# jytime/Deep-SfM-Revisited

Measured on AMD Instinct MI355X. Metric: image-pairs/sec (5-pt RANSAC + nlabel=128 plane-sweep), KITTI 376×1242, higher is better.
Workload: dtype f64+f32; 1 GPU; KITTI 376x1242 dense flow (N=435032, read by the RANSAC kernels), H=4096 hypotheses (ransac_iter=8), nlabel=128, C=32 at 94x311, fp32 cost volume; pairs_per_gpu=8, global_batch=8, parallelism=dp1, streams=one stream

## Files before the change

### deep-sfm-revisited_amd/csrc/ransac5.hip

```cpp
#include <string>
#include <vector>
#include "ransac_common.h"

namespace sfm {

template <class Src>
static int run_chunk(const Src& src, const int64_t* n, int bc, int num_test,
                     int num_ransac_test, int iters, double thr, uint64_t seed, int cheir,
                     const Workspace& w, int ws_batch, double* E_out, double* P_out, int32_t* inliers_out,
                     int32_t* winner_out, int32_t* score_out, hipStream_t s, bool first_chunk,
                     const RefJob* ref_job = nullptr, bool* rode = nullptr) {
  const int H = kChains * iters;
  const int cmax = H * kMaxSlots;
  PairParams pp{};
  for (int b = 0; b < bc; ++b) {
    pp.n[b] = n[b];
    pp.test[b] = (int32_t)(num_test > 0 ? num_test : n[b]);
    pp.rtest[b] = (int32_t)(num_ransac_test > 0 ? num_ransac_test : n[b]);
    const int M = std::max(pp.test[b], pp.rtest[b]);
    pp.splits[b] = (M + kPtsPerItem - 1) / kPtsPerItem;
  }
  const ScorePlan plan = make_score_plan(thr, pp, bc, cmax, ws_batch, score_out != nullptr, true);
  launch_solve(src, pp, bc, H, seed, cheir, w, s);
  SFM_LAUNCHED();
// ... 158 lines not shown
    set_error("workspace too small: need " + std::to_string(need) + " bytes");
    return SFM_ERR_WORKSPACE;
  }
  hipStream_t s = (hipStream_t)stream;
  char* p = (char*)workspace;
  const size_t c = (size_t)batch * ncand;
  ScoreBufs w;
  w.cand_total = (int32_t*)p;
  p += align_up(SFM_MAX_BATCH * 4);
  w.candE = (double*)p;
  p += align_up(c * kCandStride * 8);
  w.candF = (_Float16*)p;
  p += align_up(c * kMfRec * 2);
  w.cntR = (int32_t*)p;
  p += align_up(c * 4);
  w.claim = (unsigned long long*)p;
  w.cntT = counts;
  PairParams pp{};
  for (int b = 0; b < batch; ++b) {
    pp.n[b] = n[b];
    pp.test[b] = pp.rtest[b] = (int32_t)n[b];
    pp.splits[b] = (int32_t)((n[b] + kPtsPerItem - 1) / kPtsPerItem);
  }
  const ScorePlan plan = make_score_plan(thr, pp, batch, ncand, batch, false, false);
  SFM_HIP(hipMemsetAsync(w.cntT, 0, c * 4, s));
  SFM_HIP(hipMemsetAsync(w.cntR, 0, c * 4, s));
  launch_fill_cands(E, batch, ncand, thr, plan, w, s);
  ProfScope ps("score_essentials", s);
  launch_score(PackedSrc{pts, n_stride}, pp, w, plan, s);
  SFM_LAUNCHED();
  return SFM_OK;
}

int sfm_ransac5_candidate_counts(const void* workspace, size_t workspace_bytes, int batch, int iters,
                                 int32_t* counts_host) {
  SFM_REQUIRE(workspace && counts_host && batch >= 1 && batch <= SFM_MAX_BATCH && iters >= 1, "invalid arguments");
  const int bc = batch;
  SFM_REQUIRE(workspace_bytes >= layout(nullptr, bc, 0, iters, nullptr), "workspace too small");
  Workspace w;
  layout((char*)workspace, bc, 0, iters, &w);
  SFM_HIP(hipMemcpy(counts_host, w.cand_total, sizeof(int32_t) * batch, hipMemcpyDeviceToHost));
  return SFM_OK;
}

int sfm_ransac5_hypothesis_counts(const void* workspace, size_t workspace_bytes, int batch, int iters,
                                  int32_t* nroots_host, int32_t* ncand_host) {
  SFM_REQUIRE(workspace && nroots_host && ncand_host && batch >= 1 && batch <= SFM_MAX_BATCH && iters >= 1,
              "invalid arguments");
  const int bc = batch;
  SFM_REQUIRE(workspace_bytes >= layout(nullptr, bc, 0, iters, nullptr), "workspace too small");
  Workspace w;
  layout((char*)workspace, bc, 0, iters, &w);
  const size_t bytes = sizeof(int32_t) * (size_t)batch * kChains * iters;
  SFM_HIP(hipMemcpy(nroots_host, w.nroots, bytes, hipMemcpyDeviceToHost));
  SFM_HIP(hipMemcpy(ncand_host, w.ncand, bytes, hipMemcpyDeviceToHost));
  return SFM_OK;
}

int sfm_ransac5_skipped_evaluations(const void* workspace, size_t workspace_bytes, int batch, int iters,
                                    unsigned long long* skipped_host) {
  SFM_REQUIRE(workspace && skipped_host && batch >= 1 && iters >= 1, "invalid arguments");
  const int bc = std::min(batch, SFM_MAX_BATCH);
  SFM_REQUIRE(workspace_bytes >= layout(nullptr, bc, 0, iters, nullptr), "workspace too small");
  Workspace w;
  layout((char*)workspace, bc, 0, iters, &w);
  SFM_HIP(hipMemcpy(skipped_host, w.skipped, sizeof(unsigned long long), hipMemcpyDeviceToHost));
// ... 19 lines not shown
```

### deep-sfm-revisited_amd/csrc/ransac_common.h

```cpp
#pragma once
#include <algorithm>
#include "common.h"

namespace sfm {

constexpr int kChains = SFM_RANSAC_CHAINS;
constexpr int kMaxSlots = 10;
constexpr size_t kMf2ClaimBytes = 9 * sizeof(unsigned long long);
constexpr int kCandStride = 18;
constexpr int kStEb = 0, kStA = 36, kStQ = 75, kStPoly = 95, kStRoots = 106, kStateFields = 116;
constexpr int kKC = 32;
constexpr int kPPL = 8;
constexpr int kScoreThreads = 256;
constexpr int kChunk = kScoreThreads * kPPL;
constexpr int kPPL32 = 8;
constexpr int kPtsPerItem = 8192;
static_assert(kPtsPerItem % kChunk == 0, "item = whole chunks");
constexpr int kMfRec = 64;
constexpr int kMf2Span = 1024;
constexpr int kBestStride = 64;

struct PairParams {
  int64_t n[SFM_MAX_BATCH];
  int32_t test[SFM_MAX_BATCH];
// ... 153 lines not shown
  int32_t* cmap = nullptr;
  int32_t* lead = nullptr;
  unsigned long long* skipped = nullptr;
  int32_t* bnd = nullptr;
};

struct MfParams {
  int k;
  double t_lo, t_hi;
};

enum class Scorer {
  kMf2Prune,
  kMf2,
  kMf,
  kLowp,
  kScore32,
  kFma,
  kRef
};
struct ScorePlan {
  Scorer scorer;
  int bc, cmax;
  bool same;
  int prec;
  ScoreConsts kc;
  MfParams mp;
  double guard_g;
  bool fast32;
  int cus;
  int grid;
  int mf2_pm;
  bool one_cnt;
};
#pragma GCC visibility push(hidden)
ScorePlan make_score_plan(double thr, const PairParams& pp, int bc, int cmax, int ws_batch, bool want_scores,
                          bool allow_prune);
template <class Src>
void launch_score(const Src& src, const PairParams& pp, const ScoreBufs& w, const ScorePlan& plan, hipStream_t s,
                  const RefJob* ref_job = nullptr, bool* rode = nullptr);

template <class Src>
void launch_solve(const Src& src, const PairParams& pp, int bc, int H, uint64_t seed, int cheir, const Workspace& w,
                  hipStream_t s);
void launch_chain(int bc, int H, int iters, int cheir, double thr, const ScorePlan& plan, const Workspace& w,
                  bool first_chunk, hipStream_t s);
void launch_select(int bc, int H, int cheir, const ScorePlan& plan, const Workspace& w, int32_t* score_out,
                   double* E_out, double* P_out, int32_t* inliers_out, int32_t* winner_out, hipStream_t s);
void launch_fill_cands(const double* E, int batch, int ncand, double thr, const ScorePlan& plan, const ScoreBufs& w,
                       hipStream_t s);
#pragma GCC visibility pop

}
```

### deep-sfm-revisited_amd/csrc/ransac_score.hip

```cpp
#include "score_mf2.h"

namespace sfm {

template <int kFmt>
static bool make_rider(const RefJob& j, long long max_runs, RefRider<kFmt>* r) {
  const long long hw = (long long)j.h * j.w, L = j.nlabel;
  const long long esz = kFmt == 1 ? 4 : 2;
  if (hw < 4 || hw % 2 != 0 || (hw % 4 != 0 && L % 2 != 0)) return false;
  const long long P = hw % 4 == 0 ? hw : 2 * hw, np = L * hw / P;
  const long long slab_bytes = L * hw * esz;
  if (slab_bytes >= (1ll << 32) || (uintptr_t)j.ref % 8 != 0 || (uintptr_t)j.cost % 16 != 0) return false;
  const long long rows = (long long)j.batch * j.channels;
  const long long cpp = (P + 255) / 256, gpp = (np + kRiderStores - 1) / kRiderStores;
  const long long T = rows * cpp * gpp;
  if (T >= (1ll << 31) || max_runs >= (1ll << 31)) return false;
  r->ref = j.ref;
  r->cost = j.cost;
  r->T = (unsigned)T;
  r->C = (unsigned)j.channels;
  r->hw = (unsigned)hw;
  r->P = (unsigned)P;
  r->cpp = (unsigned)cpp;
  r->np = (unsigned)np;
  r->gpp = (unsigned)gpp;
// ... 2 lines not shown
  r->mgpp = make_magic((unsigned)gpp);
  r->mC = make_magic((unsigned)j.channels);
  return true;
}

static int lowp_prec() {
  const int p = tuning().score_precision;
  return (p != 64 && tuning().score_lowp_template) ? p + 1 : p;
}

ScorePlan make_score_plan(double thr, const PairParams& pp, int bc, int cmax, int ws_batch, bool want_scores,
                          bool allow_prune) {
  ScorePlan p{};
  p.bc = bc;
  p.cmax = cmax;
  p.prec = lowp_prec();
  const bool fast = p.prec == 64 && thr >= 0x1p-40 && thr < 1.0;
  p.guard_g = fast ? 0x1p24 * (11.0 + 11.0 / thr) : 0.0;
  p.fast32 = fast && thr >= 0x1p-20 && tuning().score_fp32;
  ScoreConsts& kc = p.kc;
  kc.thr = thr;
  kc.t2lo = (thr * thr) * (1.0 - 0x1p-22);
  kc.t2hi = (thr * thr) * (1.0 + 0x1p-22);
  kc.t2lo32 = (float)((thr * thr) * (1.0 - 0x1p-6 - 0x1p-19));
  kc.t2hi32 = (float)((thr * thr) * (1.0 + 0x1p-7) / (1.0 - 0x1p-7) * (1.0 + 0x1p-19));
  kc.fast32 = p.fast32 ? 1 : 0;
  kc.ws_batch = ws_batch;
  kc.interleave = tuning().score_interleave;
  int dev = 0, cus = 256;
  if (hipGetDevice(&dev) == hipSuccess) (void)hipDeviceGetAttribute(&cus, hipDeviceAttributeMultiprocessorCount, dev);
  p.cus = std::max(1, cus);
  p.grid = p.cus * tuning().score_blocks_per_cu;
  p.same = true;
  int min_spans = INT32_MAX;
  for (int b = 0; b < bc; ++b) {
    p.same = p.same && pp.test[b] == pp.rtest[b];
    min_spans = std::min(min_spans, mf2_spans(std::max(pp.test[b], pp.rtest[b])));
  }
  const bool use_mf = p.fast32 && tuning().score_mf && mf_params(thr, &p.mp);
  const bool mf2 = use_mf && p.same && tuning().score_mf == 2;
  const bool may_prune = allow_prune && p.same && !want_scores;
  kc.prune = (p.fast32 && !use_mf && may_prune && tuning().score_prune) ? 1 : 0;
  p.mf2_pm = (mf2 && may_prune && min_spans >= kMf2PruneMinSpans) ? tuning().score_mf_prune : 0;
  p.one_cnt = mf2;
  const bool lowp = p.prec == 32 || p.prec == 16 || p.prec == 33 || p.prec == 17;
  p.scorer = mf2 ? (p.mf2_pm > 0 ? Scorer::kMf2Prune : Scorer::kMf2)
             : use_mf ? Scorer::kMf
             : lowp ? Scorer::kLowp
             : p.fast32 ? Scorer::kScore32
             : fast ? Scorer::kFma
                    : Scorer::kRef;
  return p;
}

struct Mf2Launch {
  const int32_t* cand_total;
  const int32_t* cmap;
  int sp_lo, sp_hi;
  const int32_t* bnd;
  int phase;
  int chunk;
};
static Mf2Launch spans_pm(const int32_t* cand_total, int lo, int hi, int chunk, const int32_t* cmap = nullptr) {
  return Mf2Launch{cand_total, cmap, lo, hi, nullptr, 0, chunk};
}
static Mf2Launch spans_bnd(const int32_t* cand_total, const int32_t* bnd, int phase, int chunk,
                           const int32_t* cmap = nullptr) {
  return Mf2Launch{cand_total, cmap, 0, 0, bnd, phase, chunk};
}

template <class Src, bool kMapped, bool kUpper, class... Rider>
// ... 4 lines not shown
                     a.sp_lo, a.sp_hi, a.bnd, a.phase, a.chunk, rider...);
}

template <int kFmt, class Src>
static bool try_ride(const Src& src, const PairParams& pp, const ScoreBufs& w, const ScorePlan& plan, hipStream_t s,
                     const Mf2Launch& a, const RefJob* job, long long max_runs) {
  RefRider<kFmt> r;
  if (!job || !tuning().score_ref_rider || job->dtype != kFmt - 1 || !make_rider(*job, max_runs, &r)) return false;
  launch_mf2<Src, false, true>(src, pp, w, plan, s, a, r);
  return true;
}

template <class Src, bool kUpper>
static void launch_mf2_pruned(const Src& src, const PairParams& pp, const ScoreBufs& w, const ScorePlan& plan,
                              hipStream_t s, const RefJob* ref_job, bool* rode) {
  const int bc = plan.bc, cmax = plan.cmax;
  const int ch = tuning().score_mf_chunk;
  const int ch2 = tuning().score_mf_chunk2 ? tuning().score_mf_chunk2 : ch;
  const int32_t* kept = w.lead + 3 * SFM_MAX_BATCH;
  const Mf2Launch A = spans_pm(w.cand_total, 0, plan.mf2_pm, ch);
  bool ride = false;
  if constexpr (kUpper) {
    long long max_runs = 0;
    for (int b = 0; b < bc; ++b)
      max_runs += (long long)mf2_spans(std::max(pp.test[b], pp.rtest[b])) * ((cmax + kKC - 1) / kKC);
    ride = try_ride<1>(src, pp, w, plan, s, A, ref_job, max_runs) ||
           try_ride<2>(src, pp, w, plan, s, A, ref_job, max_runs);
    if (ride) *rode = true;
  }
  if (!ride) launch_mf2<Src, false, kUpper>(src, pp, w, plan, s, A);
  hipLaunchKernelGGL(k_mf2_split, dim3(bc), dim3(1024), 0, s, pp, cmax, plan.mf2_pm, tuning().score_mf_prune_margin,
                     w.cand_total, w.cntT, w.bnd, kUpper ? w.lead : nullptr);
  launch_mf2<Src, false, kUpper>(src, pp, w, plan, s, spans_bnd(w.cand_total, w.bnd, 1, ch));
  hipLaunchKernelGGL(k_mf2_lead<Src>, dim3(kUpper ? 4 * kLeadBlocks : kLeadBlocks, bc), dim3(1024), 0, s, src, pp,
                     cmax, w.bnd, w.cand_total, w.candE, w.cntT, plan.kc, w.lead, kUpper ? 2 : 0);
  hipLaunchKernelGGL(k_mf2_keep, dim3((cmax + 1023) / 1024, bc), dim3(1024), 0, s, pp, cmax, w.bnd, w.cand_total,
                     w.cntT, w.lead, w.cmap, w.skipped, 0);
  launch_mf2<Src, true, kUpper>(src, pp, w, plan, s, spans_bnd(kept, w.bnd, 2, ch2, w.cmap));
  if constexpr (kUpper) {
    const int exact_max = tuning().score_mf_exact_max;
    hipLaunchKernelGGL(k_mf2_keep_map, dim3(bc), dim3(1024), 0, s, cmax, w.cntT, w.lead, w.cmap, w.cmap2, exact_max);
    hipLaunchKernelGGL(k_mf2_zero_kept, dim3((cmax + 255) / 256, bc), dim3(256), 0, s, cmax, w.lead, w.cmap2, w.cntT);
    hipLaunchKernelGGL(k_mf2_exact<Src>, dim3(kExactBlocks, bc), dim3(kExactThreads), 0, s, src, pp, cmax, w.lead,
                       w.cmap2, w.candE, plan.kc, w.cntT, exact_max);
    launch_mf2<Src, true, false>(src, pp, w, plan, s, spans_pm(w.lead + 4 * SFM_MAX_BATCH, 0, 1000, ch2, w.cmap2));
  }
}

template <bool FAST, int PREC, class Src>
static void launch_valu(const Src& src, const PairParams& pp, const ScoreBufs& w, const ScorePlan& plan,
                        hipStream_t s, const char* name) {
  hipLaunchKernelGGL((k_score<FAST, Src, PREC>), dim3(plan.grid), dim3(kScoreThreads), 0, s, src, pp, plan.bc,
                     plan.cmax, w.cand_total, w.candE, w.cntT, w.cntR, plan.kc);
  set_last_scorer(name);
}

template <class Src>
void launch_score(const Src& src, const PairParams& pp, const ScoreBufs& w, const ScorePlan& plan, hipStream_t s,
                  const RefJob* ref_job, bool* rode) {
  const int bc = plan.bc, cmax = plan.cmax;
  if (plan.scorer <= Scorer::kMf)
    hipLaunchKernelGGL(k_mf_cands, dim3((cmax + 255) / 256, bc), dim3(256), 0, s, cmax, w.cand_total, w.candE, w.candF,
                       plan.mp, w.claim, plan.mf2_pm > 0 ? w.lead : nullptr);
  const dim3 gmf(plan.cus * tuning().score_mf_blocks_per_cu);
  switch (plan.scorer) {
    case Scorer::kMf2Prune:
      if (tuning().score_mf_prune_upper) launch_mf2_pruned<Src, true>(src, pp, w, plan, s, ref_job, rode);
      else launch_mf2_pruned<Src, false>(src, pp, w, plan, s, ref_job, rode);
      set_last_scorer("k_score_mf2+prune");
      break;
    case Scorer::kMf2:
      launch_mf2<Src, false, false>(src, pp, w, plan, s, spans_pm(w.cand_total, 0, 1000, tuning().score_mf_chunk));
      set_last_scorer("k_score_mf2");
      break;
    case Scorer::kMf:
      if (plan.same)
        hipLaunchKernelGGL((k_score_mf<Src, true>), gmf, dim3(kMfWaves * 64), 0, s, src, pp, bc, cmax, w.cand_total,
                           w.candE, w.candF, w.cntT, w.cntR, plan.kc);
      else
// ... 31 lines not shown
```

### deep-sfm-revisited_amd/csrc/score_mf2.h

```cpp
#pragma once
#include <hip/hip_bf16.h>
#include "score_mf.h"

namespace sfm {

constexpr int kMf2Waves = 12;
constexpr int kMf2Wpe = kMf2Waves / 4;
#ifndef SFM_MF2_UP_WAVES
#define SFM_MF2_UP_WAVES 16
#endif
template <bool kUpper> constexpr int mf2_waves() { return kUpper ? SFM_MF2_UP_WAVES : kMf2Waves; }
constexpr int kMf2Tiles = kMf2Span / 32;
constexpr int kMf2Guide = 2;
constexpr int kMf2Queue = 128;
#ifndef SFM_MF2_WQ
#define SFM_MF2_WQ 1
#endif
constexpr int kMf2WordSlots = kMf2Queue / 2;
constexpr int kMf2TblTiles = 352;
constexpr int kMf2TblWords = kMf2TblTiles * kKC / 2;
constexpr int kMf2TblSpans = 63;
constexpr int kMf2PruneMinSpans = 32;
static_assert(kMf2Span <= 1024, "16-bit table counts");
static_assert(kMf2Tiles <= 32 && kMf2Tiles % 2 == 0, "32-bit decision strings, tiles in pairs");
// ... 485 lines not shown
        if constexpr (kRide) {
          __builtin_amdgcn_s_waitcnt(0x0F70);
          if (rp < rp_end) {
            const auto& rj = rider_of(rider...);
            rider_store(rj, rp, lane, rd);
            for (unsigned p = rp + 1u; p < rp_end; ++p) rider_store(rj, p, lane, rider_load(rj, p, lane));
          }
        }
        k = kn;
      }
      u += k1 - k0;
      lds_barrier();
    }
  }
  if (tb >= 0) flush(tb);
  __syncthreads();
  if (tid == 0) {
    __threadfence();
    if (atomicAdd(claim + 8, 1ull) == (unsigned long long)G - 1ull) {
#pragma unroll
      for (int i = 0; i < 9; ++i) claim[i] = 0ull;
    }
  }
}

constexpr int kLeadBlocks = 32;
constexpr int kExactMaxKept = 256;

__device__ __forceinline__ int mf2_n1(const PairParams& pp, int b, const int32_t* bnd) {
  const int M = max(pp.test[b], pp.rtest[b]);
  return min(bnd[2 * SFM_MAX_BATCH + b] * kMf2Span, M);
}

__global__ __launch_bounds__(1024) void k_mf2_split(PairParams pp, int cmax, int pm, int margin,
                                                   const int32_t* __restrict__ cand_total,
                                                   const int32_t* __restrict__ cntT, int32_t* __restrict__ bnd,
                                                   int32_t* __restrict__ leader) {
  __shared__ unsigned long long s_key[16];
  const int b = blockIdx.x, tid = threadIdx.x, lane = tid & 63, wv = tid >> 6;
  const int M = max(pp.test[b], pp.rtest[b]);
  const int all = mf2_spans(M);
  const int sA = mf2_span_at(all, pm);
  const int nA = min(sA * kMf2Span, M);
  const int ctot = cand_total[b];
  const int32_t* cnt = cntT + (size_t)b * cmax;
  unsigned long long key = 0ull;
  for (int c = tid; c < ctot; c += 1024) {
    const unsigned long long k = ((unsigned long long)(uint32_t)cnt[c] << 32) | (uint32_t)(0xFFFFFFFFu - (uint32_t)c);
    key = k > key ? k : key;
  }
#pragma unroll
  for (int d = 32; d >= 1; d >>= 1) {
    const unsigned long long o = __shfl_xor(key, d, 64);
    key = o > key ? o : key;
  }
  if (lane == 0) s_key[wv] = key;
  __syncthreads();
  if (tid != 0) return;
  for (int w = 0; w < 16; ++w) key = s_key[w] > key ? s_key[w] : key;
  int mx = (int)(key >> 32);
  if (leader && ctot > 0) {
    leader[0 * SFM_MAX_BATCH + b] = 0;
    leader[1 * SFM_MAX_BATCH + b] = (int)(0xFFFFFFFFu - (uint32_t)(key & 0xFFFFFFFFull));
  }
  const long long rho_pm = nA > 0 ? ((long long)mx * 1000) / nA : 0;
  long long f = 1000 - rho_pm + margin;
  f = max(f, (long long)pm);
  const int sB = f > 990 ? all : max(sA, mf2_span_at(all, (int)f));
  bnd[0 * SFM_MAX_BATCH + b] = 0;
  bnd[1 * SFM_MAX_BATCH + b] = sA;
  bnd[2 * SFM_MAX_BATCH + b] = sB;
  bnd[3 * SFM_MAX_BATCH + b] = all;
}

template <class Src>
__global__ __launch_bounds__(1024) void k_mf2_lead(const Src src, PairParams pp, int cmax, const int32_t* __restrict__ bnd,
                                                  const int32_t* __restrict__ cand_total,
                                                  const double* __restrict__ candE, const int32_t* __restrict__ cntT,
                                                  ScoreConsts kc, int32_t* __restrict__ lead, int full) {
  __shared__ unsigned long long s_key[16];
  __shared__ int s_part[16];
  const int b = blockIdx.y, tid = threadIdx.x, lane = tid & 63, wv = tid >> 6;
  const int M = max(pp.test[b], pp.rtest[b]);
  const int n1 = full ? 0 : mf2_n1(pp, b, bnd);
  const int ctot = cand_total[b];
  if (ctot <= 0) return;
  const int32_t* cnt = cntT + (size_t)b * cmax;
  if (full == 2) {
    const int ldr = lead[1 * SFM_MAX_BATCH + b];
    const int k0 = (int)((long long)M * blockIdx.x / gridDim.x);
    const int k1 = (int)((long long)M * (blockIdx.x + 1) / gridDim.x);
    const double* El = candE + ((size_t)b * cmax + ldr) * kCandStride;
    int r = 0;
    const int T = (int)blockDim.x;
    for (int k = k0 + tid; k < k1; k += 2 * T) {
      const bool ob = k + T < k1;
      const double4 va = src.load(b, k), vb = src.load(b, ob ? k + T : k);
      r += inlier_f64v(El, va, kc) ? 1 : 0;
      r += (ob && inlier_f64v(El, vb, kc)) ? 1 : 0;
    }
#pragma unroll
    for (int d = 32; d >= 1; d >>= 1) r += __shfl_xor(r, d, 64);
    if (lane == 0) s_part[wv] = r;
    __syncthreads();
    if (tid == 0) {
      int t = 0;
      for (int w = 0; w < (int)(blockDim.x >> 6); ++w) t += s_part[w];
      if (t) atomicAdd(&lead[2 * SFM_MAX_BATCH + b], t);
    }
    return;
  }
  unsigned long long key = 0ull;
  for (int c = tid; c < ctot; c += 1024) {
    const unsigned long long k = ((unsigned long long)(uint32_t)cnt[c] << 32) | (uint32_t)(0xFFFFFFFFu - (uint32_t)c);
    key = k > key ? k : key;
  }
#pragma unroll
  for (int d = 32; d >= 1; d >>= 1) {
    const unsigned long long o = __shfl_xor(key, d, 64);
    key = o > key ? o : key;
  }
  if (lane == 0) s_key[wv] = key;
  __syncthreads();
  key = s_key[0];
  for (int w = 1; w < 16; ++w) key = s_key[w] > key ? s_key[w] : key;
  const int ld = (int)(0xFFFFFFFFu - (uint32_t)(key & 0xFFFFFFFFull));
  const int rest_n = M - n1;
  const int k0 = n1 + (int)((long long)rest_n * blockIdx.x / gridDim.x);
  const int k1 = n1 + (int)((long long)rest_n * (blockIdx.x + 1) / gridDim.x);
  const double* El = candE + ((size_t)b * cmax + ld) * kCandStride;
  int rest = 0;
  for (int k = k0 + tid; k < k1; k += 1024) rest += inlier_f64v(El, src.load(b, k), kc) ? 1 : 0;
#pragma unroll
  for (int d = 32; d >= 1; d >>= 1) rest += __shfl_xor(rest, d, 64);
  if (lane == 0) s_part[wv] = rest;
  __syncthreads();
  if (tid == 0) {
    int r = 0;
    for (int w = 0; w < 16; ++w) r += s_part[w];
    if (blockIdx.x == 0) {
      lead[0 * SFM_MAX_BATCH + b] = full ? 0 : (int)(key >> 32);
      lead[1 * SFM_MAX_BATCH + b] = ld;
// ... 21 lines not shown
  int before = 0;
  for (int c = tid; c < c0; c += 1024) before += kept(c) ? 1 : 0;
#pragma unroll
  for (int d = 32; d >= 1; d >>= 1) before += __shfl_xor(before, d, 64);
  const int c = c0 + tid;
  const bool keep = c < ctot && kept(c);
  const unsigned long long bal = __ballot(keep);
  if (lane == 0) {
    s_part[wv] = __popcll(bal);
    s_before[wv] = before;
  }
  __syncthreads();
  int base = 0, tot = 0;
  for (int w = 0; w < 16; ++w) {
    base += s_before[w];
    tot += s_part[w];
  }
  if (keep) {
    int off = base + __popcll(bal & ((1ull << lane) - 1ull));
    for (int w = 0; w < wv; ++w) off += s_part[w];
    cmap[(size_t)b * cmax + off] = c;
  }
  if (tid == 0) {
    if (c0 + 1024 >= ctot) {
      lead[3 * SFM_MAX_BATCH + b] = base + tot;
      lead[4 * SFM_MAX_BATCH + b] = base + tot > exact_max ? base + tot : 0;
    }
    const int live = min(1024, ctot - c0);
    if (skipped && live > tot)
      atomicAdd(skipped, (unsigned long long)(live - tot) * (unsigned long long)(M - n1));
  }
}

constexpr int kExactBlocks = 128;
constexpr int kExactThreads = 1024;

template <class Src>
__global__ __launch_bounds__(kExactThreads) void k_mf2_exact(const Src src, PairParams pp, int cmax,
                                                   const int32_t* __restrict__ lead, const int32_t* __restrict__ cmap,
                                                   const double* __restrict__ candE, ScoreConsts kc,
                                                   int32_t* __restrict__ cntT, int exact_max) {
  __shared__ int32_t s_cnt[kExactMaxKept];
  __shared__ double s_E[kExactMaxKept][10];
  const int b = blockIdx.y, tid = threadIdx.x;
  const int kept = lead[3 * SFM_MAX_BATCH + b];
  if (kept <= 0 || kept > exact_max) return;
  const int32_t* mp = cmap + (size_t)b * cmax;
  const double* Eb = candE + (size_t)b * cmax * kCandStride;
  for (int c = tid; c < kept; c += kExactThreads) s_cnt[c] = 0;
  for (int i = tid; i < kept * 10; i += kExactThreads) s_E[i / 10][i % 10] = Eb[(size_t)mp[i / 10] * kCandStride + i % 10];
  __syncthreads();
  const int M = max(pp.test[b], pp.rtest[b]);
  const int k0 = (int)((long long)M * blockIdx.x / gridDim.x);
  const int k1 = (int)((long long)M * (blockIdx.x + 1) / gridDim.x);
  const int lane = tid & 63;
  for (int base = k0; base < k1; base += 2 * kExactThreads) {
    const int ka = base + tid, kb = base + kExactThreads + tid;
    const bool oa = ka < k1, ob = kb < k1;
    const double4 va = src.load(b, oa ? ka : k0), vb = src.load(b, ob ? kb : k0);
#pragma unroll 1
    for (int j = 0; j < kept; ++j) {
      const bool ia = inlier_f64v(&s_E[j][0], va, kc), ib = inlier_f64v(&s_E[j][0], vb, kc);
      const int n = (int)__popcll(__ballot(oa && ia)) + (int)__popcll(__ballot(ob && ib));
      if (lane == 0 && n) atomicAdd(&s_cnt[j], n);
    }
  }
  __syncthreads();
  for (int c = tid; c < kept; c += kExactThreads)
    if (s_cnt[c]) atomicAdd(cntT + (size_t)b * cmax + mp[c], s_cnt[c]);
}

__global__ __launch_bounds__(1024) void k_mf2_keep_map(int cmax, const int32_t* __restrict__ cntT,
                                                      int32_t* __restrict__ lead, const int32_t* __restrict__ cmap_in,
                                                      int32_t* __restrict__ cmap_out, int exact_max) {
  __shared__ int s_part[16];
  __shared__ int s_base;
  const int b = blockIdx.x, tid = threadIdx.x, lane = tid & 63, wv = tid >> 6;
  const int n = lead[3 * SFM_MAX_BATCH + b];
  const long long lb = (long long)lead[0 * SFM_MAX_BATCH + b] + lead[2 * SFM_MAX_BATCH + b];
  const int32_t* cnt = cntT + (size_t)b * cmax;
  const int32_t* in = cmap_in + (size_t)b * cmax;
  int32_t* out = cmap_out + (size_t)b * cmax;
  if (tid == 0) s_base = 0;
  __syncthreads();
  for (int j0 = 0; j0 < n; j0 += 1024) {
    const int j = j0 + tid;
    const int c = j < n ? in[j] : 0;
    const bool keep = j < n && (long long)cnt[c] >= lb;
    const unsigned long long bal = __ballot(keep);
    if (lane == 0) s_part[wv] = __popcll(bal);
    __syncthreads();
    int off = s_base + __popcll(bal & ((1ull << lane) - 1ull));
    for (int w = 0; w < wv; ++w) off += s_part[w];
    if (keep) out[off] = c;
    __syncthreads();
    if (tid == 0) {
      int t = 0;
      for (int w = 0; w < 16; ++w) t += s_part[w];
      s_base += t;
    }
    __syncthreads();
  }
// ... 15 lines not shown
```

### deep-sfm-revisited_amd/sfm_amd/_lib.py

```python
import ctypes
import os

_HERE = os.path.dirname(os.path.abspath(__file__))
LIB_PATH = os.environ.get("SFM_HIP_LIB") or os.path.join(_HERE, "libsfm_hip.so")

_c_dp = ctypes.c_void_p
_i64p = ctypes.POINTER(ctypes.c_int64)

_SIGS = [
    ("sfm_abi_version", ctypes.c_int, []),
    ("sfm_last_error", ctypes.c_char_p, []),
    ("sfm_ransac5_workspace_bytes", ctypes.c_size_t, [ctypes.c_int, ctypes.c_int64, ctypes.c_int]),
    ("sfm_ransac5", ctypes.c_int,
     [_c_dp, _c_dp, ctypes.c_int64, ctypes.c_int, ctypes.c_int, ctypes.c_int, ctypes.c_double,
      ctypes.c_uint64, ctypes.c_int, _c_dp, ctypes.c_size_t, _c_dp, _c_dp, _c_dp, _c_dp, _c_dp]),
    ("sfm_ransac5_packed", ctypes.c_int,
     [_c_dp, ctypes.c_int64, _i64p, ctypes.c_int, ctypes.c_int, ctypes.c_int, ctypes.c_int,
      ctypes.c_double, ctypes.c_uint64, ctypes.c_int, _c_dp, ctypes.c_size_t, _c_dp, _c_dp, _c_dp, _c_dp,
      _c_dp, _c_dp]),
    ("sfm_ransac5_inlier_mask", ctypes.c_int,
     [_c_dp, ctypes.c_int64, _i64p, ctypes.c_int, _c_dp, ctypes.c_double, _c_dp, _c_dp]),
    ("sfm_flow_to_points", ctypes.c_int,
     [_c_dp, ctypes.c_int, ctypes.c_int, ctypes.c_int, ctypes.c_int, ctypes.c_int, ctypes.c_int, _c_dp, _c_dp,
      _c_dp]),
# ... 139 lines not shown
    ("sfm_context_unpack_grad_f16", ctypes.c_int,
     [_c_dp, _c_dp, ctypes.c_int, ctypes.c_int, ctypes.c_int, ctypes.c_int, ctypes.c_int, ctypes.c_int, ctypes.c_int,
      _c_dp, _c_dp, _c_dp]),
    ("sfm_dep_context_pack_f16", ctypes.c_int,
     [_c_dp, _c_dp, ctypes.c_int, _c_dp, ctypes.c_int, ctypes.c_int, ctypes.c_int, ctypes.c_int, ctypes.c_int,
      ctypes.c_int, ctypes.c_int, ctypes.c_int, _c_dp, _c_dp]),
    ("sfm_dep_context_pack_bf16", ctypes.c_int,
     [_c_dp, _c_dp, ctypes.c_int, _c_dp, ctypes.c_int, ctypes.c_int, ctypes.c_int, ctypes.c_int, ctypes.c_int,
      ctypes.c_int, ctypes.c_int, ctypes.c_int, _c_dp, _c_dp]),
    ("sfm_dep_context_unpack_grad_f16", ctypes.c_int,
     [_c_dp, ctypes.c_int, ctypes.c_int, ctypes.c_int, ctypes.c_int, ctypes.c_int, ctypes.c_int, ctypes.c_int,
      ctypes.c_int, _c_dp, _c_dp]),
    ("sfm_conv2x_f16", ctypes.c_int,
     [_c_dp, ctypes.c_int, ctypes.c_int, ctypes.c_int, ctypes.c_int, _c_dp, ctypes.c_int, ctypes.c_int, ctypes.c_int,
      ctypes.c_int, _c_dp, _c_dp, ctypes.c_int, _c_dp, _c_dp, _c_dp]),
    ("sfm_conv2x_wgrad_f16_workspace_bytes", ctypes.c_size_t,
     [ctypes.c_int, ctypes.c_int, ctypes.c_int, ctypes.c_int, ctypes.c_int, ctypes.c_int, ctypes.c_int]),
    ("sfm_conv2x_wgrad_f16", ctypes.c_int,
     [_c_dp, _c_dp, ctypes.c_int, ctypes.c_int, ctypes.c_int, ctypes.c_int, ctypes.c_int, ctypes.c_int, ctypes.c_int,
      ctypes.c_int, _c_dp, _c_dp, ctypes.c_size_t, _c_dp]),
    ("sfm_conv2x_dgrad_f16", ctypes.c_int,
     [_c_dp, ctypes.c_int, ctypes.c_int, ctypes.c_int, ctypes.c_int, _c_dp, ctypes.c_int, ctypes.c_int, ctypes.c_int,
      ctypes.c_int, ctypes.c_int, ctypes.c_int, _c_dp, _c_dp]),
    ("sfm_image_pack_f16", ctypes.c_int, [_c_dp, ctypes.c_int, ctypes.c_int, ctypes.c_int, _c_dp, _c_dp]),
    ("sfm_avgpool_f16", ctypes.c_int,
     [_c_dp, ctypes.c_int, ctypes.c_int, ctypes.c_int, ctypes.c_int, ctypes.c_int, _c_dp, _c_dp]),
    ("sfm_spp_pack_f16", ctypes.c_int,
     [_c_dp, _c_dp, ctypes.POINTER(ctypes.c_void_p), ctypes.POINTER(ctypes.c_int), ctypes.POINTER(ctypes.c_int),
      ctypes.c_int, ctypes.c_int, ctypes.c_int, _c_dp, _c_dp]),
    ("sfm_score_essentials_workspace_bytes", ctypes.c_size_t, [ctypes.c_int, ctypes.c_int]),
    ("sfm_score_essentials", ctypes.c_int,
     [_c_dp, ctypes.c_int64, _i64p, ctypes.c_int, _c_dp, ctypes.c_int, ctypes.c_double, _c_dp, _c_dp,
      ctypes.c_size_t, _c_dp]),
    ("sfm_tune_set", ctypes.c_int, [ctypes.c_char_p, ctypes.c_int]),
    ("sfm_tune_get", ctypes.c_int, [ctypes.c_char_p, ctypes.POINTER(ctypes.c_int)]),
    ("sfm_tune_key", ctypes.c_char_p, [ctypes.c_int]),
    ("sfm_last_scorer", ctypes.c_char_p, []),
    ("sfm_last_sweep", ctypes.c_char_p, []),
    ("sfm_profile_enable", ctypes.c_int, [ctypes.c_int]),
    ("sfm_profile_select", ctypes.c_int, [ctypes.c_char_p]),
    ("sfm_profile_reset", ctypes.c_int, []),
    ("sfm_profile_read", ctypes.c_int,
     [ctypes.c_char_p, ctypes.POINTER(ctypes.c_double), ctypes.POINTER(ctypes.c_int)]),
]

SYMBOLS = [s[0] for s in _SIGS]

_lib = None
_load_error = None


class SfmError(RuntimeError):
    pass


def load():
    global _lib, _load_error
    if _lib is not None:
        return _lib
    if not os.path.exists(LIB_PATH):
        raise SfmError(f"libsfm_hip.so not found at {LIB_PATH}: build it with "
                       f"`make -C deep-sfm-revisited_amd/csrc` (or __graft_entry__.build())")
    try:
        lib = ctypes.CDLL(LIB_PATH)
    except OSError as e:
        _load_error = e
# ... 87 lines not shown
```

### deep-sfm-revisited_amd/sfm_amd/ransac.py

```python
import torch

from . import _lib

CHAINS = 512
DEFAULT_SEED = 1234


def _check_dev_f64(t, name):
    if not t.is_cuda:
        raise RuntimeError(f"{name} must be a CUDA tensor")
    if t.dtype != torch.float64:
        raise RuntimeError(f"{name} must be a double tensor")
    if not t.is_contiguous():
        raise RuntimeError(f"{name} must be contiguous")


def _flow_and_kinv(flow, intrinsic_inv):
    if not flow.is_cuda:
        raise RuntimeError("flow must be a CUDA tensor")
    if flow.dim() != 4 or flow.shape[1] != 2:
        raise RuntimeError(f"flow must be [B,2,H,W], got {tuple(flow.shape)}")
    B = flow.shape[0]
    return flow.contiguous().float(), _kinv_batch(intrinsic_inv, B, flow.device)

# ... 66 lines not shown
def ransac5_batched(pts, n=None, num_test_points=None, num_ransac_test_points=None, iters=5, threshold=1e-4,
                    seed=DEFAULT_SEED, cheirality=True, return_scores=False, workspace=None, precision=64):
    if int(precision) != 64:
        with score_precision(precision):
            return ransac5_batched(pts, n, num_test_points, num_ransac_test_points, iters, threshold, seed,
                                   cheirality, return_scores, workspace)
    _check_dev_f64(pts, "pts")
    if pts.dim() != 3 or pts.shape[2] != 4:
        raise RuntimeError("pts must be [B, N, 4]")
    B, ns, _ = pts.shape
    n = [ns] * B if n is None else [int(v) for v in n]
    if len(n) != B:
        raise RuntimeError("len(n) must equal the batch size")
    dev = pts.device
    H = hypotheses(iters)
    with torch.cuda.device(dev):
        if workspace is None:
            workspace = _workspace(B, 0, iters, dev)
        E = torch.empty(B, 3, 3, dtype=torch.float64, device=dev)
        P = torch.empty(B, 3, 4, dtype=torch.float64, device=dev) if cheirality else None
        inl = torch.empty(B, dtype=torch.int32, device=dev)
        win = torch.empty(B, dtype=torch.int32, device=dev)
        scores = torch.empty(B, H, dtype=torch.int32, device=dev) if return_scores else None
        rc = _lib.load().sfm_ransac5_packed(
            _lib.ptr(pts), ns, _lib.i64_array(n), B, int(num_test_points or 0), int(num_ransac_test_points or 0),
            int(iters), float(threshold), int(seed), 1 if cheirality else 0, _lib.ptr(workspace),
            workspace.numel(), _lib.ptr(E), _lib.ptr(P), _lib.ptr(inl), _lib.ptr(win), _lib.ptr(scores),
            _lib.stream_ptr(dev))
        _lib.check(rc, "sfm_ransac5_packed")
    out = (E, P, inl, win)
    return out + (scores,) if return_scores else out


def score_essentials(pts, E, threshold, n=None):
    _check_dev_f64(pts, "pts")
    B, ns, _ = pts.shape
    n = [ns] * B if n is None else [int(v) for v in n]
    E = E.reshape(B, -1, 9).to(pts.device, torch.float64).contiguous()
    C = E.shape[1]
    L = _lib.load()
    counts = torch.empty(B, C, dtype=torch.int32, device=pts.device)
    with torch.cuda.device(pts.device):
        ws = torch.empty(int(L.sfm_score_essentials_workspace_bytes(B, C)), dtype=torch.uint8, device=pts.device)
        _lib.check(L.sfm_score_essentials(_lib.ptr(pts), ns, _lib.i64_array(n), B, _lib.ptr(E), C, float(threshold),
                                          _lib.ptr(counts), _lib.ptr(ws), ws.numel(), _lib.stream_ptr(pts.device)),
                   "sfm_score_essentials")
    return counts


def workspace_for(batch, iters, device):
    return _workspace(batch, 0, iters, device)


def pack_points(q, qp):
    _check_dev_f64(q, "input1")
    _check_dev_f64(qp, "input2")
    n = q.shape[0]
    out = torch.empty(1, n, 4, dtype=torch.float64, device=q.device)
    with torch.cuda.device(q.device):
        _lib.check(_lib.load().sfm_pack_points(_lib.ptr(q), _lib.ptr(qp), n, _lib.ptr(out),
                                               _lib.stream_ptr(q.device)), "sfm_pack_points")
    return out


def inlier_mask(pts, E, threshold, n=None):
    _check_dev_f64(pts, "pts")
    B, ns, _ = pts.shape
    n = [ns] * B if n is None else [int(v) for v in n]
    E = E.reshape(B, 9).contiguous().to(torch.float64)
    mask = torch.empty(B, ns, dtype=torch.uint8, device=pts.device)
    with torch.cuda.device(pts.device):
        _lib.check(_lib.load().sfm_ransac5_inlier_mask(_lib.ptr(pts), ns, _lib.i64_array(n), B, _lib.ptr(E),
                                                       float(threshold), _lib.ptr(mask),
                                                       _lib.stream_ptr(pts.device)), "sfm_ransac5_inlier_mask")
    return mask.bool()


def flow_to_points(flow, intrinsic_inv, h_side=None, w_side=None, margin=10, out=None):
    flow, Ki = _flow_and_kinv(flow, intrinsic_inv)
# ... 172 lines not shown
```

### include/sfm_hip.h

```cpp
#ifndef SFM_HIP_H
#define SFM_HIP_H

#include <stddef.h>
#include <stdint.h>

#ifdef __cplusplus
extern "C" {
#endif

enum {
  SFM_OK = 0,
  SFM_ERR_ARG = 1,
  SFM_ERR_HIP = 2,
  SFM_ERR_WORKSPACE = 3
};

#define SFM_ABI_VERSION 1
#define SFM_RANSAC_CHAINS 512
#define SFM_MAX_BATCH 64

int sfm_abi_version(void);
const char* sfm_last_error(void);


size_t sfm_ransac5_workspace_bytes(int batch, int64_t n_max, int iters);

int sfm_ransac5(const double* q, const double* qp, int64_t n,
                int num_test, int num_ransac_test, int iters, double thr,
                uint64_t seed, int cheirality,
                void* workspace, size_t workspace_bytes,
                double* E_out, double* P_out, int32_t* inliers_out, int32_t* winner_out,
                void* stream);

int sfm_ransac5_packed(const double* pts, int64_t n_stride, const int64_t* n, int batch,
                       int num_test, int num_ransac_test, int iters, double thr,
                       uint64_t seed, int cheirality,
                       void* workspace, size_t workspace_bytes,
                       double* E_out, double* P_out, int32_t* inliers_out, int32_t* winner_out,
                       int32_t* hyp_score_out, void* stream);

int sfm_ransac5_flow(const float* flow, int batch, int H, int W, int h_side, int w_side, int margin,
                     const float* Kinv, int num_test, int num_ransac_test, int iters, double thr,
                     uint64_t seed, int cheirality, void* workspace, size_t workspace_bytes,
                     double* E_out, double* P_out, int32_t* inliers_out, int32_t* winner_out,
                     int32_t* hyp_score_out, void* stream);

size_t sfm_score_essentials_workspace_bytes(int batch, int ncand);
int sfm_score_essentials(const double* pts, int64_t n_stride, const int64_t* n, int batch, const double* E,
                         int ncand, double thr, int32_t* counts, void* workspace, size_t workspace_bytes,
                         void* stream);

int sfm_ransac5_inlier_mask(const double* pts, int64_t n_stride, const int64_t* n, int batch,
                            const double* E, double thr, uint8_t* mask, void* stream);

int sfm_flow_to_points(const float* flow, int batch, int H, int W, int h_side, int w_side,
                       int margin, const float* Kinv, double* pts_out, void* stream);

int sfm_keypoints_to_points(const float* flow, int batch, int H, int W, int h_side, int w_side,
                            const float* kp1, const float* kp2, int64_t kp_stride, const int64_t* n, int mode,
                            const float* Kinv, double* pts_out, int64_t n_stride, void* stream);

int sfm_ransac5_candidate_counts(const void* workspace, size_t workspace_bytes, int batch, int iters,
                                 int32_t* counts_host);

int sfm_ransac5_hypothesis_counts(const void* workspace, size_t workspace_bytes, int batch, int iters,
                                  int32_t* nroots_host, int32_t* ncand_host);

int sfm_ransac5_skipped_evaluations(const void* workspace, size_t workspace_bytes, int batch, int iters,
                                    unsigned long long* skipped_host);
int sfm_ransac5_kept_candidates(const void* workspace, size_t workspace_bytes, int batch, int iters,
                                int32_t* kept_host, int32_t* points_host);

int sfm_pack_points(const double* q, const double* qp, int64_t n, double* pts_out, void* stream);

int sfm_essential_optimise(const double* q, const double* qp, int64_t n, const double* E_init,
                           double delta, double alpha, int max_reps, double* E_out);
size_t sfm_essential_optimise_workspace_bytes(int batch, int64_t n_max);
int sfm_essential_optimise_batched(const double* pts, int64_t n_stride, const int64_t* n, int batch,
                                   const double* E_init, double delta, double alpha, int max_reps,
                                   double* E_out, void* workspace, size_t workspace_bytes, void* stream);
int sfm_essential_decompose(const double* E, double* params5);
int sfm_essential_decompose_uv(const double* E, double* U, double* V);

// ... 203 lines not shown
```

Measured before the change: 1955 pairs/s.

## Unify lead/exact counting into a shared chunked 256-thread count kernel

Replaces the fixed-grid 1024-thread leader and exact inlier-count kernels with one shared device routine. It runs 256-thread blocks, each loading four points per thread and working over a point chunk sized from the total point count and CU count. The grid now scales with the number of points rather than being fixed at 128 or 4×kLeadBlocks blocks, which is meant to improve occupancy and memory-level parallelism. It also adds an exact-count API entry point for testing. In exchange it launches more blocks and does more shared-memory atomics per block.

```diff
diff --git a/deep-sfm-revisited_amd/csrc/ransac5.hip b/deep-sfm-revisited_amd/csrc/ransac5.hip
--- a/deep-sfm-revisited_amd/csrc/ransac5.hip
+++ b/deep-sfm-revisited_amd/csrc/ransac5.hip
@@ -214,6 +214,44 @@
   return SFM_OK;
 }
 
+int sfm_count_essentials_exact(const double* pts, int64_t n_stride, const int64_t* n, int batch, const double* E,
+                               int ncand, double thr, int32_t* counts, void* workspace, size_t workspace_bytes,
+                               void* stream) {
+  SFM_REQUIRE(pts && n && E && counts, "null pointer argument");
+  SFM_REQUIRE(batch >= 1 && batch <= SFM_MAX_BATCH, "batch must be in [1, 64]");
+  SFM_REQUIRE(ncand >= 1 && ncand <= 256, "ncand must be in [1, 256]");
+  SFM_REQUIRE(thr >= 0x1p-40 && thr < 1.0, "inlier threshold must be in [2^-40, 1)");
+  SFM_REQUIRE(n_stride >= 1 && n_stride <= (int64_t)INT32_MAX, "n_stride out of range");
+  for (int b = 0; b < batch; ++b) SFM_REQUIRE(n[b] >= 1 && n[b] <= n_stride, "each n[b] must be in [1, n_stride]");
+  const size_t need = sfm_score_essentials_workspace_bytes(batch, ncand);
+  if (!workspace || workspace_bytes < need) {
+    set_error("workspace too small: need " + std::to_string(need) + " bytes");
+    return SFM_ERR_WORKSPACE;
+  }
+  hipStream_t s = (hipStream_t)stream;
+  char* p = (char*)workspace;
+  const size_t c = (size_t)batch * ncand;
+  ScoreBufs w;
+  w.cand_total = (int32_t*)p;
+  p += align_up(SFM_MAX_BATCH * 4);
+  w.candE = (double*)p;
+  p += align_up(c * kCandStride * 8) + align_up(c * kMfRec * 2);
+  w.cntR = (int32_t*)p;
+  w.cntT = counts;
+  PairParams pp{};
+  for (int b = 0; b < batch; ++b) {
+    pp.n[b] = n[b];
+    pp.test[b] = pp.rtest[b] = (int32_t)n[b];
+  }
+  const ScorePlan plan = make_score_plan(thr, pp, batch, ncand, batch, true, false);
+  SFM_HIP(hipMemsetAsync(w.cntT, 0, c * 4, s));
+  launch_fill_cands(E, batch, ncand, thr, plan, w, s);
+  ProfScope ps("count_exact", s);
+  launch_count_exact(PackedSrc{pts, n_stride}, pp, w, plan, s);
+  SFM_LAUNCHED();
+  return SFM_OK;
+}
+
 int sfm_ransac5_candidate_counts(const void* workspace, size_t workspace_bytes, int batch, int iters,
                                  int32_t* counts_host) {
   SFM_REQUIRE(workspace && counts_host && batch >= 1 && batch <= SFM_MAX_BATCH && iters >= 1, "invalid arguments");
diff --git a/deep-sfm-revisited_amd/csrc/ransac_common.h b/deep-sfm-revisited_amd/csrc/ransac_common.h
--- a/deep-sfm-revisited_amd/csrc/ransac_common.h
+++ b/deep-sfm-revisited_amd/csrc/ransac_common.h
@@ -209,6 +209,7 @@
   int grid;
   int mf2_pm;
   bool one_cnt;
+  int lead_chunk, lead_grid, exact_chunk, exact_grid;
 };
 #pragma GCC visibility push(hidden)
 ScorePlan make_score_plan(double thr, const PairParams& pp, int bc, int cmax, int ws_batch, bool want_scores,
@@ -216,6 +217,9 @@
 template <class Src>
 void launch_score(const Src& src, const PairParams& pp, const ScoreBufs& w, const ScorePlan& plan, hipStream_t s,
                   const RefJob* ref_job = nullptr, bool* rode = nullptr);
+
+void launch_count_exact(const PackedSrc& src, const PairParams& pp, const ScoreBufs& w, const ScorePlan& plan,
+                        hipStream_t s);
 
 template <class Src>
 void launch_solve(const Src& src, const PairParams& pp, int bc, int H, uint64_t seed, int cheir, const Workspace& w,
diff --git a/deep-sfm-revisited_amd/csrc/ransac_score.hip b/deep-sfm-revisited_amd/csrc/ransac_score.hip
--- a/deep-sfm-revisited_amd/csrc/ransac_score.hip
+++ b/deep-sfm-revisited_amd/csrc/ransac_score.hip
@@ -58,11 +58,19 @@
   p.cus = std::max(1, cus);
   p.grid = p.cus * tuning().score_blocks_per_cu;
   p.same = true;
-  int min_spans = INT32_MAX;
+  int min_spans = INT32_MAX, max_pts = 1;
+  long long pts = 0;
   for (int b = 0; b < bc; ++b) {
     p.same = p.same && pp.test[b] == pp.rtest[b];
     min_spans = std::min(min_spans, mf2_spans(std::max(pp.test[b], pp.rtest[b])));
-  }
+    max_pts = std::max(max_pts, std::max(pp.test[b], pp.rtest[b]));
+    pts += std::max(pp.test[b], pp.rtest[b]);
+  }
+  const long long lead_pts = (pts / (4ll * p.cus) + kCountPass - 1) / kCountPass * kCountPass;
+  p.lead_chunk = (int)std::min<long long>(std::max<long long>(lead_pts, kCountPass), 8 * kCountPass);
+  p.exact_chunk = kCountPass;
+  p.lead_grid = (int)(((long long)max_pts + p.lead_chunk - 1) / p.lead_chunk);
+  p.exact_grid = (int)(((long long)max_pts + p.exact_chunk - 1) / p.exact_chunk);
   const bool use_mf = p.fast32 && tuning().score_mf && mf_params(thr, &p.mp);
   const bool mf2 = use_mf && p.same && tuning().score_mf == 2;
   const bool may_prune = allow_prune && p.same && !want_scores;
@@ -133,8 +141,9 @@
   hipLaunchKernelGGL(k_mf2_split, dim3(bc), dim3(1024), 0, s, pp, cmax, plan.mf2_pm, tuning().score_mf_prune_margin,
                      w.cand_total, w.cntT, w.bnd, kUpper ? w.lead : nullptr);
   launch_mf2<Src, false, kUpper>(src, pp, w, plan, s, spans_bnd(w.cand_total, w.bnd, 1, ch));
-  hipLaunchKernelGGL(k_mf2_lead<Src>, dim3(kUpper ? 4 * kLeadBlocks : kLeadBlocks, bc), dim3(1024), 0, s, src, pp,
-                     cmax, w.bnd, w.cand_total, w.candE, w.cntT, plan.kc, w.lead, kUpper ? 2 : 0);
+  hipLaunchKernelGGL(k_mf2_lead<Src>, dim3(kUpper ? plan.lead_grid : kLeadBlocks, bc),
+                     dim3(kUpper ? kCountThreads : 1024), 0, s, src, pp, cmax, w.bnd, w.cand_total, w.candE, w.cntT,
+                     plan.kc, w.lead, kUpper ? 2 : 0, plan.lead_chunk);
   hipLaunchKernelGGL(k_mf2_keep, dim3((cmax + 1023) / 1024, bc), dim3(1024), 0, s, pp, cmax, w.bnd, w.cand_total,
                      w.cntT, w.lead, w.cmap, w.skipped, 0);
   launch_mf2<Src, true, kUpper>(src, pp, w, plan, s, spans_bnd(kept, w.bnd, 2, ch2, w.cmap));
@@ -142,10 +151,17 @@
     const int exact_max = tuning().score_mf_exact_max;
     hipLaunchKernelGGL(k_mf2_keep_map, dim3(bc), dim3(1024), 0, s, cmax, w.cntT, w.lead, w.cmap, w.cmap2, exact_max);
     hipLaunchKernelGGL(k_mf2_zero_kept, dim3((cmax + 255) / 256, bc), dim3(256), 0, s, cmax, w.lead, w.cmap2, w.cntT);
-    hipLaunchKernelGGL(k_mf2_exact<Src>, dim3(kExactBlocks, bc), dim3(kExactThreads), 0, s, src, pp, cmax, w.lead,
-                       w.cmap2, w.candE, plan.kc, w.cntT, exact_max);
+    hipLaunchKernelGGL(k_mf2_exact<Src>, dim3(plan.exact_grid, bc), dim3(kCountThreads), 0, s, src, pp, cmax,
+                       plan.exact_chunk, kept, w.cmap2, w.candE, plan.kc, w.cntT, exact_max);
     launch_mf2<Src, true, false>(src, pp, w, plan, s, spans_pm(w.lead + 4 * SFM_MAX_BATCH, 0, 1000, ch2, w.cmap2));
   }
+}
+
+void launch_count_exact(const PackedSrc& src, const PairParams& pp, const ScoreBufs& w, const ScorePlan& plan,
+                        hipStream_t s) {
+  hipLaunchKernelGGL(k_iota_list, dim3((plan.cmax + 255) / 256, plan.bc), dim3(256), 0, s, plan.cmax, w.cntR);
+  hipLaunchKernelGGL(k_mf2_exact<PackedSrc>, dim3(plan.exact_grid, plan.bc), dim3(kCountThreads), 0, s, src, pp,
+                     plan.cmax, plan.exact_chunk, w.cand_total, w.cntR, w.candE, plan.kc, w.cntT, kExactMaxKept);
 }
 
 template <bool FAST, int PREC, class Src>
diff --git a/deep-sfm-revisited_amd/csrc/score_mf2.h b/deep-sfm-revisited_amd/csrc/score_mf2.h
--- a/deep-sfm-revisited_amd/csrc/score_mf2.h
+++ b/deep-sfm-revisited_amd/csrc/score_mf2.h
@@ -541,6 +541,50 @@
   return min(bnd[2 * SFM_MAX_BATCH + b] * kMf2Span, M);
 }
 
+constexpr int kCountThreads = 256;
+constexpr int kCountChains = 4;
+constexpr int kCountPass = kCountThreads * kCountChains;
+
+template <class Src, int kMaxList, bool kSlot>
+__device__ __forceinline__ void mf2_count_list(const Src& src, const PairParams& pp, int b, int chunk,
+                                               const int32_t* __restrict__ list, int n_list,
+                                               const double* __restrict__ Eb, const ScoreConsts& kc,
+                                               int32_t* __restrict__ out) {
+  __shared__ int32_t s_cnt[kMaxList];
+  __shared__ double s_E[kMaxList][10];
+  const int tid = threadIdx.x, lane = tid & 63;
+  const int M = max(pp.test[b], pp.rtest[b]);
+  const long long first = (long long)blockIdx.x * chunk;
+  if (first >= M) return;
+  const int k0 = (int)first, rem = (int)min((long long)chunk, (long long)M - first);
+  for (int c = tid; c < n_list; c += kCountThreads) s_cnt[c] = 0;
+  for (int i = tid; i < n_list * 10; i += kCountThreads) s_E[i / 10][i % 10] = Eb[(size_t)list[i / 10] * kCandStride + i % 10];
+  __syncthreads();
+  for (int off = tid; off - tid < rem; off += kCountPass) {
+    double4 v[kCountChains];
+    bool on[kCountChains];
+#pragma unroll
+    for (int c = 0; c < kCountChains; ++c) {
+      const int o = off + c * kCountThreads;
+      on[c] = o < rem;
+      v[c] = src.load(b, k0 + (on[c] ? o : 0));
+    }
+#pragma unroll 1
+    for (int j = 0; j < n_list; ++j) {
+      int n = 0;
+#pragma unroll
+      for (int c = 0; c < kCountChains; ++c) {
+        const bool in = inlier_f64v(&s_E[j][0], v[c], kc);
+        n += (int)__popcll(__ballot(on[c] && in));
+      }
+      if (lane == 0 && n) atomicAdd(&s_cnt[j], n);
+    }
+  }
+  __syncthreads();
+  for (int c = tid; c < n_list; c += kCountThreads)
+    if (s_cnt[c]) atomicAdd(out + (kSlot ? list[c] : 0), s_cnt[c]);
+}
+
 __global__ __launch_bounds__(1024) void k_mf2_split(PairParams pp, int cmax, int pm, int margin,
                                                    const int32_t* __restrict__ cand_total,
                                                    const int32_t* __restrict__ cntT, int32_t* __restrict__ bnd,
@@ -586,7 +630,7 @@
 __global__ __launch_bounds__(1024) void k_mf2_lead(const Src src, PairParams pp, int cmax, const int32_t* __restrict__ bnd,
                                                   const int32_t* __restrict__ cand_total,
                                                   const double* __restrict__ candE, const int32_t* __restrict__ cntT,
-                                                  ScoreConsts kc, int32_t* __restrict__ lead, int full) {
+                                                  ScoreConsts kc, int32_t* __restrict__ lead, int full, int chunk) {
   __shared__ unsigned long long s_key[16];
   __shared__ int s_part[16];
   const int b = blockIdx.y, tid = threadIdx.x, lane = tid & 63, wv = tid >> 6;
@@ -596,27 +640,8 @@
   if (ctot <= 0) return;
   const int32_t* cnt = cntT + (size_t)b * cmax;
   if (full == 2) {
-    const int ldr = lead[1 * SFM_MAX_BATCH + b];
-    const int k0 = (int)((long long)M * blockIdx.x / gridDim.x);
-    const int k1 = (int)((long long)M * (blockIdx.x + 1) / gridDim.x);
-    const double* El = candE + ((size_t)b * cmax + ldr) * kCandStride;
-    int r = 0;
-    const int T = (int)blockDim.x;
-    for (int k = k0 + tid; k < k1; k += 2 * T) {
-      const bool ob = k + T < k1;
-      const double4 va = src.load(b, k), vb = src.load(b, ob ? k + T : k);
-      r += inlier_f64v(El, va, kc) ? 1 : 0;
-      r += (ob && inlier_f64v(El, vb, kc)) ? 1 : 0;
-    }
-#pragma unroll
-    for (int d = 32; d >= 1; d >>= 1) r += __shfl_xor(r, d, 64);
-    if (lane == 0) s_part[wv] = r;
-    __syncthreads();
-    if (tid == 0) {
-      int t = 0;
-      for (int w = 0; w < (int)(blockDim.x >> 6); ++w) t += s_part[w];
-      if (t) atomicAdd(&lead[2 * SFM_MAX_BATCH + b], t);
-    }
+    mf2_count_list<Src, 1, false>(src, pp, b, chunk, lead + 1 * SFM_MAX_BATCH + b, 1,
+                                  candE + (size_t)b * cmax * kCandStride, kc, lead + 2 * SFM_MAX_BATCH + b);
     return;
   }
   unsigned long long key = 0ull;
@@ -704,42 +729,21 @@
   }
 }
 
-constexpr int kExactBlocks = 128;
-constexpr int kExactThreads = 1024;
-
 template <class Src>
-__global__ __launch_bounds__(kExactThreads) void k_mf2_exact(const Src src, PairParams pp, int cmax,
-                                                   const int32_t* __restrict__ lead, const int32_t* __restrict__ cmap,
+__global__ __launch_bounds__(kCountThreads) void k_mf2_exact(const Src src, PairParams pp, int cmax, int chunk,
+                                                   const int32_t* __restrict__ n_list, const int32_t* __restrict__ cmap,
                                                    const double* __restrict__ candE, ScoreConsts kc,
                                                    int32_t* __restrict__ cntT, int exact_max) {
-  __shared__ int32_t s_cnt[kExactMaxKept];
-  __shared__ double s_E[kExactMaxKept][10];
-  const int b = blockIdx.y, tid = threadIdx.x;
-  const int kept = lead[3 * SFM_MAX_BATCH + b];
+  const int b = blockIdx.y;
+  const int kept = n_list[b];
   if (kept <= 0 || kept > exact_max) return;
-  const int32_t* mp = cmap + (size_t)b * cmax;
-  const double* Eb = candE + (size_t)b * cmax * kCandStride;
-  for (int c = tid; c < kept; c += kExactThreads) s_cnt[c] = 0;
-  for (int i = tid; i < kept * 10; i += kExactThreads) s_E[i / 10][i % 10] = Eb[(size_t)mp[i / 10] * kCandStride + i % 10];
-  __syncthreads();
-  const int M = max(pp.test[b], pp.rtest[b]);
-  const int k0 = (int)((long long)M * blockIdx.x / gridDim.x);
-  const int k1 = (int)((long long)M * (blockIdx.x + 1) / gridDim.x);
-  const int lane = tid & 63;
-  for (int base = k0; base < k1; base += 2 * kExactThreads) {
-    const int ka = base + tid, kb = base + kExactThreads + tid;
-    const bool oa = ka < k1, ob = kb < k1;
-    const double4 va = src.load(b, oa ? ka : k0), vb = src.load(b, ob ? kb : k0);
-#pragma unroll 1
-    for (int j = 0; j < kept; ++j) {
-      const bool ia = inlier_f64v(&s_E[j][0], va, kc), ib = inlier_f64v(&s_E[j][0], vb, kc);
-      const int n = (int)__popcll(__ballot(oa && ia)) + (int)__popcll(__ballot(ob && ib));
-      if (lane == 0 && n) atomicAdd(&s_cnt[j], n);
-    }
-  }
-  __syncthreads();
-  for (int c = tid; c < kept; c += kExactThreads)
-    if (s_cnt[c]) atomicAdd(cntT + (size_t)b * cmax + mp[c], s_cnt[c]);
+  mf2_count_list<Src, kExactMaxKept, true>(src, pp, b, chunk, cmap + (size_t)b * cmax, kept,
+                                           candE + (size_t)b * cmax * kCandStride, kc, cntT + (size_t)b * cmax);
+}
+
+__global__ __launch_bounds__(256) void k_iota_list(int n, int32_t* __restrict__ list) {
+  const int i = (int)(blockIdx.x * 256 + threadIdx.x);
+  if (i < n) list[(size_t)blockIdx.y * n + i] = i;
 }
 
 __global__ __launch_bounds__(1024) void k_mf2_keep_map(int cmax, const int32_t* __restrict__ cntT,
diff --git a/deep-sfm-revisited_amd/sfm_amd/_lib.py b/deep-sfm-revisited_amd/sfm_amd/_lib.py
--- a/deep-sfm-revisited_amd/sfm_amd/_lib.py
+++ b/deep-sfm-revisited_amd/sfm_amd/_lib.py
@@ -195,6 +195,9 @@
     ("sfm_score_essentials", ctypes.c_int,
      [_c_dp, ctypes.c_int64, _i64p, ctypes.c_int, _c_dp, ctypes.c_int, ctypes.c_double, _c_dp, _c_dp,
       ctypes.c_size_t, _c_dp]),
+    ("sfm_count_essentials_exact", ctypes.c_int,
+     [_c_dp, ctypes.c_int64, _i64p, ctypes.c_int, _c_dp, ctypes.c_int, ctypes.c_double, _c_dp, _c_dp,
+      ctypes.c_size_t, _c_dp]),
     ("sfm_tune_set", ctypes.c_int, [ctypes.c_char_p, ctypes.c_int]),
     ("sfm_tune_get", ctypes.c_int, [ctypes.c_char_p, ctypes.POINTER(ctypes.c_int)]),
     ("sfm_tune_key", ctypes.c_char_p, [ctypes.c_int]),
diff --git a/deep-sfm-revisited_amd/sfm_amd/ransac.py b/deep-sfm-revisited_amd/sfm_amd/ransac.py
--- a/deep-sfm-revisited_amd/sfm_amd/ransac.py
+++ b/deep-sfm-revisited_amd/sfm_amd/ransac.py
@@ -122,7 +122,7 @@
     return out + (scores,) if return_scores else out
 
 
-def score_essentials(pts, E, threshold, n=None):
+def score_essentials(pts, E, threshold, n=None, exact_list=False):
     _check_dev_f64(pts, "pts")
     B, ns, _ = pts.shape
     n = [ns] * B if n is None else [int(v) for v in n]
@@ -132,9 +132,10 @@
     counts = torch.empty(B, C, dtype=torch.int32, device=pts.device)
     with torch.cuda.device(pts.device):
         ws = torch.empty(int(L.sfm_score_essentials_workspace_bytes(B, C)), dtype=torch.uint8, device=pts.device)
-        _lib.check(L.sfm_score_essentials(_lib.ptr(pts), ns, _lib.i64_array(n), B, _lib.ptr(E), C, float(threshold),
-                                          _lib.ptr(counts), _lib.ptr(ws), ws.numel(), _lib.stream_ptr(pts.device)),
-                   "sfm_score_essentials")
+        fn = L.sfm_count_essentials_exact if exact_list else L.sfm_score_essentials
+        _lib.check(fn(_lib.ptr(pts), ns, _lib.i64_array(n), B, _lib.ptr(E), C, float(threshold), _lib.ptr(counts),
+                      _lib.ptr(ws), ws.numel(), _lib.stream_ptr(pts.device)),
+                   "sfm_count_essentials_exact" if exact_list else "sfm_score_essentials")
     return counts
 
 
diff --git a/include/sfm_hip.h b/include/sfm_hip.h
--- a/include/sfm_hip.h
+++ b/include/sfm_hip.h
@@ -49,6 +49,10 @@
 int sfm_score_essentials(const double* pts, int64_t n_stride, const int64_t* n, int batch, const double* E,
                          int ncand, double thr, int32_t* counts, void* workspace, size_t workspace_bytes,
                          void* stream);
+
+int sfm_count_essentials_exact(const double* pts, int64_t n_stride, const int64_t* n, int batch, const double* E,
+                               int ncand, double thr, int32_t* counts, void* workspace, size_t workspace_bytes,
+                               void* stream);
 
 int sfm_ransac5_inlier_mask(const double* pts, int64_t n_stride, const int64_t* n, int batch,
                             const double* E, double thr, uint8_t* mask, void* stream);
```

Measured after the change: 1956 pairs/s (median of 3 runs). About the same (+0.1%).
